# PolySummit/SCORP

Hardware: AMD Instinct MI355X
Metric: fwd+bwd views/sec @1M Gaussians 1600x1200 SH3 (higher is better)
Workload: dtype f32; 1 GPU; S3: 1000000 Gaussians, 1600x1200, SH degree 3, ring cameras (SURVEY 8d); views_per_rank=116, distinct_cameras_per_rank=280, views_in_flight=1, pairs_per_view_D=2428534, visible=966997, parallelism=view-sharded replicas x1

## Files before the change

### scorp_amd/csrc/loss.hip

```cpp
#include "common.hpp"

namespace scorp {
namespace {

constexpr int kLT = 32;
constexpr int kLH = 5;
constexpr int kLP = kLT + 2 * kLH;
constexpr int kLPS = kLP + 3;
constexpr int kLHS = kLT + 1;
constexpr int kHO = 6;
constexpr int kHG = (kLT + kHO - 1) / kHO;
constexpr float kC1 = 0.01f * 0.01f, kC2 = 0.03f * 0.03f;

struct Window { float w[11]; };

Window make_window() {
  Window win;
  float s = 0.0f;
  for (int i = 0; i < 11; i++) { win.w[i] = (float)exp(-(double)((i - 5) * (i - 5)) / (2.0 * 1.5 * 1.5)); s += win.w[i]; }
  for (int i = 0; i < 11; i++) win.w[i] /= s;
  return win;
}

__device__ __forceinline__ float block_sum_256(float v, float *s_red) {
#pragma unroll
  for (int off = 32; off >= 1; off >>= 1) v += __shfl_xor(v, off, 64);
  const int wave = threadIdx.x >> 6;
  __syncthreads();
  if ((threadIdx.x & 63) == 0) s_red[wave] = v;
  __syncthreads();
  return s_red[0] + s_red[1] + s_red[2] + s_red[3];
}

struct LossTile { int ch, x0, y0, logical; bool valid; };
__device__ __forceinline__ LossTile loss_tile(int gx, int gy, int C) {
  const int total = gx * gy * C, per = (total + 7) / 8;
  const int b = blockIdx.x, logical = (b & 7) * per + (b >> 3);
  LossTile t;
  t.valid = (b >> 3) < per && logical < total;
  t.logical = logical;
  t.ch = logical / (gx * gy);
  const int rem = logical - t.ch * gx * gy;
  t.y0 = (rem / gx) * kLT; t.x0 = (rem % gx) * kLT;
  return t;
}

#ifndef SCORP_LOSS_STRIP_ITERS
#define SCORP_LOSS_STRIP_ITERS 3
#endif
constexpr int kStripIters = SCORP_LOSS_STRIP_ITERS;
constexpr int kStripRows = 11 * kStripIters - 10;
constexpr int kRowBuf = 80;

struct StripJob { int ch, cx0, ry0; bool valid; };
__device__ __forceinline__ StripJob strip_job(int C, int H, int W) {
  const int sx = (W + 63) / 64, sy = (H + kStripRows - 1) / kStripRows;
  const int wave = blockIdx.x * 4 + __builtin_amdgcn_readfirstlane((int)(threadIdx.x >> 6));
  StripJob j;
  j.valid = wave < C * sx * sy;
  j.ch = wave / (sx * sy);
  const int rem = wave - j.ch * sx * sy;
  j.ry0 = (rem / sx) * kStripRows; j.cx0 = (rem % sx) * 64;
  return j;
}
static inline int strip_waves(int C, int H, int W) { return C * ((W + 63) / 64) * ((H + kStripRows - 1) / kStripRows); }

__global__ void __launch_bounds__(256)
ssim_l1_forward_strip_kernel(const float *__restrict__ img, const float *__restrict__ gt, const float *__restrict__ mask,
                             int C, int H, int W, Window win, float *__restrict__ dmaps, float *__restrict__ partials) {
  __shared__ __attribute__((aligned(16))) float4 s_row4[4][kRowBuf];
  const StripJob job = strip_job(C, H, W);
  if (!job.valid) return;
  const int lane = threadIdx.x & 63, wv = __builtin_amdgcn_readfirstlane((int)(threadIdx.x >> 6));
  float4 *buf4 = s_row4[wv];
  const int ch = job.ch, cx0 = job.cx0, ry0 = job.ry0;
  const size_t HW = (size_t)H * W, CHW = (size_t)C * HW;
  const float *xp = img + ch * HW, *yp = gt + ch * HW;
  const int gx = cx0 + lane;
  const int ca = cx0 - kLH + lane, cb = cx0 + 64 - kLH + lane;
  const bool cin_a = ca >= 0 && ca < W, cin_b = lane < 2 * kLH && cb < W;
  const int ca_c = min(max(ca, 0), W - 1), cb_c = min(cb, W - 1);
  struct RowRegs { float xa, ya, ma, xb, yb, mb; };
  const uint32_t oa = (uint32_t)ca_c, ob = (uint32_t)cb_c;
  auto fetch = [&](int r) {
    RowRegs v;
    const size_t ro = (size_t)min(max(r, 0), H - 1) * W;
    const float *xr = xp + ro, *yr = yp + ro;
    v.xa = xr[oa]; v.ya = yr[oa]; v.xb = xr[ob]; v.yb = yr[ob];
    v.ma = v.mb = 1.0f;
    if (mask) { const float *mr = mask + ro; v.ma = mr[oa]; v.mb = mr[ob]; }
    return v;
  };
  const int rbeg = ry0 - kLH;
  if (mask) {
    bool any = false;
    {
      constexpr int kSupport = kStripRows + 2 * kLH;
      float ma[kSupport], mb[kSupport];
#pragma unroll
      for (int u = 0; u < kSupport; u++) {
        const float *mr = mask + (size_t)min(max(rbeg + u, 0), H - 1) * W;
        ma[u] = mr[oa]; mb[u] = mr[ob];
      }
#pragma unroll
      for (int u = 0; u < kSupport; u++) any |= (cin_a & (ma[u] != 0.0f)) | (cin_b & (mb[u] != 0.0f));
    }
    if (__ballot(any) == 0) {
      float c1 = kC1, c2 = kC2, zero = 0.0f;
      asm volatile("" : "+v"(c1), "+v"(c2), "+v"(zero));
      const float m1 = zero, m2 = zero, ess = zero, e12 = zero;
      const float m1s = m1 * m1, m2s = m2 * m2, m12 = m1 * m2;
      const float s12 = e12 - m12;
      const float A1 = 2 * m12 + c1, A2 = 2 * s12 + c2, B1 = m1s + m2s + c1, B2 = (ess - m1s - m2s) + c2;
      const float rB2 = __builtin_amdgcn_rcpf(B2);
      const float inv = __builtin_amdgcn_rcpf(B1) * rB2;
      const float ssim = A1 * A2 * inv;
      float ssim_sum = 0.0f;
      for (int ro = ry0; ro < min(ry0 + kStripRows, H); ro++) {
        if (gx < W) {
          ssim_sum += ssim;
          if (dmaps) {
            float *d0 = dmaps + ch * HW + (size_t)ro * W;
            d0[(uint32_t)gx] = (2 * m2 * (A2 - A1) - 2 * m1 * ssim * (B2 - B1)) * inv;
            (d0 + CHW)[(uint32_t)gx] = -ssim * rB2;
            (d0 + 2 * CHW)[(uint32_t)gx] = 2 * A1 * inv;
          }
        }
      }
#pragma unroll
      for (int off = 32; off >= 1; off >>= 1) ssim_sum += __shfl_xor(ssim_sum, off, 64);
      if (lane == 0) {
        const int wave = blockIdx.x * 4 + wv;
        partials[2 * wave] = 0.0f;
        partials[2 * wave + 1] = ssim_sum;
      }
      return;
    }
  }
  float hist[4][11], cx[11], cy[11];
#pragma unroll
  for (int k = 0; k < 11; k++) { hist[0][k] = hist[1][k] = hist[2][k] = hist[3][k] = 0.0f; cx[k] = cy[k] = 0.0f; }
  float l1_sum = 0.0f, ssim_sum = 0.0f;
  RowRegs n0 = fetch(rbeg), n1 = fetch(rbeg + 1);
#pragma unroll 1
  for (int it = 0; it < kStripIters; it++) {
#pragma unroll
    for (int u = 0; u < 11; u++) {
      const int r = rbeg + it * 11 + u;
      const RowRegs cur = n0;
      n0 = n1;
      n1 = fetch(r + 2);
      const bool rin = r >= 0 && r < H;
      {
        const float m = (rin && cin_a) ? cur.ma : 0.0f;
        const float xv = cur.xa * m, yv = cur.ya * m;
        buf4[lane] = make_float4(xv, yv, xv * xv + yv * yv, xv * yv);
        if (lane < 2 * kLH) {
          const float m2 = (rin && cin_b) ? cur.mb : 0.0f;
          const float x2 = cur.xb * m2, y2 = cur.yb * m2;
          buf4[64 + lane] = make_float4(x2, y2, x2 * x2 + y2 * y2, x2 * y2);
        }
      }
      __builtin_amdgcn_fence(__ATOMIC_ACQ_REL, "wavefront");
      __builtin_amdgcn_wave_barrier();
      float h0 = 0, h1 = 0, h2 = 0, h3 = 0;
#pragma unroll
      for (int k = 0; k < 11; k++) {
        const float w = win.w[k];
        const float4 b = buf4[lane + k];
        h0 += w * b.x; h1 += w * b.y; h2 += w * b.z; h3 += w * b.w;
        if (k == kLH) { cx[u] = b.x; cy[u] = b.y; }
      }
      __builtin_amdgcn_fence(__ATOMIC_ACQ_REL, "wavefront");
      __builtin_amdgcn_wave_barrier();
      hist[0][u] = h0; hist[1][u] = h1; hist[2][u] = h2; hist[3][u] = h3;
      const int ro = r - kLH;
      if (ro >= ry0 && ro < H && ro < ry0 + kStripRows) {
        float m1 = 0, m2 = 0, ess = 0, e12 = 0;
#pragma unroll
        for (int k = 0; k < 11; k++) {
          const float w = win.w[k];
          const int sl = (u + 1 + k) % 11;
          m1 += w * hist[0][sl]; m2 += w * hist[1][sl]; ess += w * hist[2][sl]; e12 += w * hist[3][sl];
        }
        if (gx < W) {
          const float m1s = m1 * m1, m2s = m2 * m2, m12 = m1 * m2;
          const float s12 = e12 - m12;
          const float A1 = 2 * m12 + kC1, A2 = 2 * s12 + kC2, B1 = m1s + m2s + kC1, B2 = (ess - m1s - m2s) + kC2;
          const float rB2 = __builtin_amdgcn_rcpf(B2);
          const float inv = __builtin_amdgcn_rcpf(B1) * rB2;
          const float ssim = A1 * A2 * inv;
          ssim_sum += ssim;
          const int sc = (u + 11 - kLH) % 11;
          l1_sum += fabsf(cx[sc] - cy[sc]);
          if (dmaps) {
            float *d0 = dmaps + ch * HW + (size_t)ro * W;
            d0[(uint32_t)gx] = (2 * m2 * (A2 - A1) - 2 * m1 * ssim * (B2 - B1)) * inv;
            (d0 + CHW)[(uint32_t)gx] = -ssim * rB2;
            (d0 + 2 * CHW)[(uint32_t)gx] = 2 * A1 * inv;
          }
        }
      }
    }
  }
#pragma unroll
  for (int off = 32; off >= 1; off >>= 1) { l1_sum += __shfl_xor(l1_sum, off, 64); ssim_sum += __shfl_xor(ssim_sum, off, 64); }
  if (lane == 0) {
    const int wave = blockIdx.x * 4 + wv;
    partials[2 * wave] = l1_sum;
    partials[2 * wave + 1] = ssim_sum;
  }
}

template <int kThreads>
__device__ __forceinline__ void finalize_sums(const float *__restrict__ partials, int nblocks, double n_elems, float lambda,
                                              float *__restrict__ out, double *s_a, double *s_b) {
  const float2 *p2 = reinterpret_cast<const float2 *>(partials);
  double a = 0, b = 0;
  for (int i0 = threadIdx.x; i0 < nblocks; i0 += 4 * kThreads) {
    float2 v[4];
#pragma unroll
    for (int j = 0; j < 4; j++) { const int i = i0 + kThreads * j; v[j] = i < nblocks ? p2[i] : make_float2(0.0f, 0.0f); }
#pragma unroll
    for (int j = 0; j < 4; j++) { a += v[j].x; b += v[j].y; }
  }
  s_a[threadIdx.x] = a; s_b[threadIdx.x] = b;
  __syncthreads();
  for (int off = kThreads / 2; off >= 1; off >>= 1) {
    if ((int)threadIdx.x < off) { s_a[threadIdx.x] += s_a[threadIdx.x + off]; s_b[threadIdx.x] += s_b[threadIdx.x + off]; }
    __syncthreads();
  }
  if (threadIdx.x == 0) {
    const double l1 = s_a[0] / n_elems, ss = s_b[0] / n_elems;
    out[0] = (float)((1.0 - lambda) * l1 + lambda * (1.0 - ss));
    out[1] = (float)l1;
    out[2] = (float)ss;
  }
}

__global__ void __launch_bounds__(1024)
loss_finalize_kernel(const float *__restrict__ partials, int nblocks, double n_elems, float lambda, float *__restrict__ out) {
  __shared__ double s_a[1024], s_b[1024];
  finalize_sums<1024>(partials, nblocks, n_elems, lambda, out, s_a, s_b);
}

struct LossFinalize { const float *partials; int nparts; double n_elems; float *out; };

template <bool kMasked>
__global__ void __launch_bounds__(256)
ssim_l1_backward_kernel(const float *__restrict__ img, const float *__restrict__ gt, const float *__restrict__ mask,
                        const float *__restrict__ dmaps, int C, int H, int W, Window win, float lambda, float inv_n,
                        const float *__restrict__ grad_out, float *__restrict__ grad_img, LossFinalize fin) {
  __shared__ __attribute__((aligned(16))) float s_m[kLP][kLPS];
  __shared__ __attribute__((aligned(16))) float s_h[kLP][kLHS];
  if (fin.out && blockIdx.x == gridDim.x - 1) {
    static_assert(sizeof(s_m) >= 256 * sizeof(double) && sizeof(s_h) >= 256 * sizeof(double), "the tree's scratch fits the tile buffers");
    finalize_sums<256>(fin.partials, fin.nparts, fin.n_elems, lambda, fin.out, reinterpret_cast<double *>(&s_m[0][0]),
                       reinterpret_cast<double *>(&s_h[0][0]));
    return;
  }
  const LossTile lt = loss_tile((W + kLT - 1) / kLT, (H + kLT - 1) / kLT, C);
  if (!lt.valid) return;
  const int ch = lt.ch, x0 = lt.x0, y0 = lt.y0;
  const size_t HW = (size_t)H * W, CHW = (size_t)C * HW;
  const int c = threadIdx.x % kLT, r0 = (threadIdx.x / kLT) * 4;
  const float go = grad_out ? grad_out[0] : 1.0f;
  float xv[4], yv[4], mk[4], acc[4];
  if constexpr (kMasked) {
#pragma unroll
    for (int o = 0; o < 4; o++) {
      const int gy = y0 + r0 + o, gx = x0 + c;
      const float m = mask[(size_t)min(gy, H - 1) * W + min(gx, W - 1)];
      mk[o] = (gy < H && gx < W) ? m : 0.0f;
    }
    const bool any = (mk[0] != 0.0f) | (mk[1] != 0.0f) | (mk[2] != 0.0f) | (mk[3] != 0.0f);
    int *s_any = reinterpret_cast<int *>(&s_h[0][0]);
    if (threadIdx.x == 0) *s_any = 0;
    __syncthreads();
    if (any) *s_any = 1;
    __syncthreads();
    const bool some = *s_any != 0;
    __syncthreads();
    if (!some) {
#pragma unroll
      for (int o = 0; o < 4; o++) {
        const int gy = y0 + r0 + o, gx = x0 + c;
        if (gy < H && gx < W) grad_img[ch * HW + (size_t)gy * W + gx] = 0.0f;
      }
      return;
    }
  } else {
#pragma unroll
    for (int o = 0; o < 4; o++) mk[o] = (y0 + r0 + o < H && x0 + c < W) ? 1.0f : 0.0f;
  }
#pragma unroll
  for (int o = 0; o < 4; o++) {
    const int gy = y0 + r0 + o, gx = x0 + c;
    const size_t p = (size_t)min(gy, H - 1) * W + min(gx, W - 1);
    xv[o] = img[ch * HW + p]; yv[o] = gt[ch * HW + p];
  }
#pragma unroll
  for (int o = 0; o < 4; o++) {
    xv[o] *= mk[o]; yv[o] *= mk[o];
    acc[o] = 0.0f;
  }
  constexpr int kPerThread = (kLP * kLP + 255) / 256;
  float pre[kPerThread];
  auto fetch = [&](int q) {
    const float *map = dmaps + q * CHW + ch * HW;
#pragma unroll
    for (int j = 0; j < kPerThread; j++) {
      const int i = min(threadIdx.x + 256 * j, kLP * kLP - 1);
      const int r = i / kLP, cc = i - r * kLP;
      const int gy = y0 + r - kLH, gx = x0 + cc - kLH;
      pre[j] = map[(size_t)min(max(gy, 0), H - 1) * W + min(max(gx, 0), W - 1)];
    }
  };
  bool pre_in[kPerThread];
#pragma unroll
  for (int j = 0; j < kPerThread; j++) {
    const int i = min(threadIdx.x + 256 * j, kLP * kLP - 1);
    const int r = i / kLP, cc = i - r * kLP;
    const int gy = y0 + r - kLH, gx = x0 + cc - kLH;
    pre_in[j] = gy >= 0 && gy < H && gx >= 0 && gx < W;
  }
  fetch(0);
#pragma unroll 1
  for (int q = 0; q < 3; q++) {
#pragma unroll
    for (int j = 0; j < kPerThread; j++) {
      const int i = threadIdx.x + 256 * j;
      if (i < kLP * kLP) s_m[i / kLP][i % kLP] = pre_in[j] ? pre[j] : 0.0f;
    }
    if (q < 2) fetch(q + 1);
    __syncthreads();
    {
      const int it = threadIdx.x;
      const int r = it / kHG, c0 = (it % kHG) * kHO;
      if (it < kLP * kHG) {
        float v[kHO + 10];
#pragma unroll
        for (int k = 0; k < kHO + 10; k++) v[k] = c0 + k < kLP ? s_m[r][c0 + k] : 0.0f;
#pragma unroll
        for (int o = 0; o < kHO; o++) {
          float sacc = 0;
#pragma unroll
          for (int k = 0; k < 11; k++) sacc += win.w[k] * v[o + k];
          if (c0 + o < kLT) s_h[r][c0 + o] = sacc;
        }
      }
    }
    __syncthreads();
    float col[14];
#pragma unroll
    for (int k = 0; k < 14; k++) col[k] = s_h[r0 + k][c];
#pragma unroll
    for (int o = 0; o < 4; o++) {
      float cv = 0;
#pragma unroll
      for (int k = 0; k < 11; k++) cv += win.w[k] * col[o + k];
      acc[o] += q == 0 ? cv : (q == 1 ? 2.0f * xv[o] * cv : yv[o] * cv);
    }
  }
#pragma unroll
  for (int o = 0; o < 4; o++) {
    const int gy = y0 + r0 + o, gx = x0 + c;
    if (gy < H && gx < W) {
      const float diff = xv[o] - yv[o];
      const float sgn = diff > 0.0f ? 1.0f : (diff < 0.0f ? -1.0f : 0.0f);
      const float g = (1.0f - lambda) * sgn - lambda * acc[o];
      grad_img[ch * HW + (size_t)gy * W + gx] = go * inv_n * mk[o] * g;
    }
  }
}

}
}

using namespace scorp;

static inline int loss_blocks(int C, int H, int W) { return ((W + kLT - 1) / kLT) * ((H + kLT - 1) / kLT) * C; }

extern "C" size_t scorp_loss_workspace_bytes(int32_t C, int32_t H, int32_t W) {
  return align_up((size_t)3 * C * H * W * 4, 256) + align_up((size_t)strip_waves(C, H, W) * 8, 256);
}

namespace scorp {
int loss_forward_impl(const float *img, const float *gt, const float *mask, int32_t C, int32_t H, int32_t W, float lambda_dssim,
                      float *out_loss3, void *workspace, size_t workspace_bytes, int32_t need_backward, bool finalize,
                      hipStream_t stream) {
  if (!img || !gt || !out_loss3 || !workspace) { set_error("NULL argument to scorp_loss_l1_ssim_forward"); return SCORP_ERR_INVALID; }
  if (C <= 0 || H <= 0 || W <= 0) { set_error("bad image shape"); return SCORP_ERR_INVALID; }
  if (workspace_bytes < scorp_loss_workspace_bytes(C, H, W) || ((uintptr_t)workspace & 15)) {
    set_error("loss workspace too small or misaligned"); return SCORP_ERR_INVALID;
  }
  float *dmaps = (float *)workspace;
  float *partials = (float *)((char *)workspace + align_up((size_t)3 * C * H * W * 4, 256));
  const Window win = make_window();
  const int nparts = strip_waves(C, H, W);
  {
    ProfScope prof(kKLossForward, stream);
    ssim_l1_forward_strip_kernel<<<(nparts + 3) / 4, 256, 0, stream>>>(img, gt, mask, C, H, W, win, need_backward ? dmaps : nullptr, partials);
  }
  SCORP_KERNEL_CHECK("ssim_l1_forward", 0, stream);
  if (finalize) {
    loss_finalize_kernel<<<1, 1024, 0, stream>>>(partials, nparts, (double)C * H * W, lambda_dssim, out_loss3);
    SCORP_KERNEL_CHECK("loss_finalize", 0, stream);
  }
  return SCORP_OK;
}

int loss_backward_impl(const float *img, const float *gt, const float *mask, int32_t C, int32_t H, int32_t W, float lambda_dssim,
                       const void *workspace, const float *grad_out, float *grad_img, float *out_loss3, hipStream_t stream) {
  if (!img || !gt || !workspace || !grad_img) { set_error("NULL argument to scorp_loss_l1_ssim_backward"); return SCORP_ERR_INVALID; }
  const int grid = (loss_blocks(C, H, W) + 7) / 8 * 8;
  const Window win = make_window();
  LossFinalize fin;
  fin.partials = (const float *)((const char *)workspace + align_up((size_t)3 * C * H * W * 4, 256));
  fin.nparts = strip_waves(C, H, W);
  fin.n_elems = (double)C * H * W;
  fin.out = out_loss3;
  {
    ProfScope prof(kKLossBackward, stream);
    if (mask)
      ssim_l1_backward_kernel<true><<<grid + (out_loss3 ? 1 : 0), 256, 0, stream>>>(img, gt, mask, (const float *)workspace, C, H, W, win,
                                                                           lambda_dssim, (float)(1.0 / ((double)C * H * W)), grad_out,
                                                                           grad_img, fin);
    else
      ssim_l1_backward_kernel<false><<<grid + (out_loss3 ? 1 : 0), 256, 0, stream>>>(img, gt, mask, (const float *)workspace, C, H, W, win,
                                                                           lambda_dssim, (float)(1.0 / ((double)C * H * W)), grad_out,
                                                                           grad_img, fin);
  }
  SCORP_KERNEL_CHECK("ssim_l1_backward", 0, stream);
  return SCORP_OK;
}
}

extern "C" int scorp_loss_l1_ssim_forward(const float *img, const float *gt, const float *mask, int32_t C, int32_t H,
                                          int32_t W, float lambda_dssim, float *out_loss3, void *workspace,
                                          size_t workspace_bytes, int32_t need_backward, scorp_stream_t stream_) {
  return loss_forward_impl(img, gt, mask, C, H, W, lambda_dssim, out_loss3, workspace, workspace_bytes, need_backward, true,
                           (hipStream_t)stream_);
}

extern "C" int scorp_loss_l1_ssim_backward(const float *img, const float *gt, const float *mask, int32_t C, int32_t H,
                                           int32_t W, float lambda_dssim, const void *workspace, const float *grad_out,
                                           float *grad_img, scorp_stream_t stream_) {
  return loss_backward_impl(img, gt, mask, C, H, W, lambda_dssim, workspace, grad_out, grad_img, nullptr, (hipStream_t)stream_);
}
```

Baseline: 1386 views/s.

## Rewrite SSIM backward as per-wave row-streaming strip kernel with rolling history

```diff
diff --git a/scorp_amd/csrc/loss.hip b/scorp_amd/csrc/loss.hip
--- a/scorp_amd/csrc/loss.hip
+++ b/scorp_amd/csrc/loss.hip
@@ -3,13 +3,7 @@
 namespace scorp {
 namespace {
 
-constexpr int kLT = 32;
 constexpr int kLH = 5;
-constexpr int kLP = kLT + 2 * kLH;
-constexpr int kLPS = kLP + 3;
-constexpr int kLHS = kLT + 1;
-constexpr int kHO = 6;
-constexpr int kHG = (kLT + kHO - 1) / kHO;
 constexpr float kC1 = 0.01f * 0.01f, kC2 = 0.03f * 0.03f;
 
 struct Window { float w[11]; };
@@ -32,19 +26,6 @@
   return s_red[0] + s_red[1] + s_red[2] + s_red[3];
 }
 
-struct LossTile { int ch, x0, y0, logical; bool valid; };
-__device__ __forceinline__ LossTile loss_tile(int gx, int gy, int C) {
-  const int total = gx * gy * C, per = (total + 7) / 8;
-  const int b = blockIdx.x, logical = (b & 7) * per + (b >> 3);
-  LossTile t;
-  t.valid = (b >> 3) < per && logical < total;
-  t.logical = logical;
-  t.ch = logical / (gx * gy);
-  const int rem = logical - t.ch * gx * gy;
-  t.y0 = (rem / gx) * kLT; t.x0 = (rem % gx) * kLT;
-  return t;
-}
-
 #ifndef SCORP_LOSS_STRIP_ITERS
 #define SCORP_LOSS_STRIP_ITERS 3
 #endif
@@ -53,9 +34,9 @@
 constexpr int kRowBuf = 80;
 
 struct StripJob { int ch, cx0, ry0; bool valid; };
-__device__ __forceinline__ StripJob strip_job(int C, int H, int W) {
+__device__ __forceinline__ StripJob strip_job(int wg, int C, int H, int W) {
   const int sx = (W + 63) / 64, sy = (H + kStripRows - 1) / kStripRows;
-  const int wave = blockIdx.x * 4 + __builtin_amdgcn_readfirstlane((int)(threadIdx.x >> 6));
+  const int wave = wg * 4 + __builtin_amdgcn_readfirstlane((int)(threadIdx.x >> 6));
   StripJob j;
   j.valid = wave < C * sx * sy;
   j.ch = wave / (sx * sy);
@@ -69,7 +50,7 @@
 ssim_l1_forward_strip_kernel(const float *__restrict__ img, const float *__restrict__ gt, const float *__restrict__ mask,
                              int C, int H, int W, Window win, float *__restrict__ dmaps, float *__restrict__ partials) {
   __shared__ __attribute__((aligned(16))) float4 s_row4[4][kRowBuf];
-  const StripJob job = strip_job(C, H, W);
+  const StripJob job = strip_job(blockIdx.x, C, H, W);
   if (!job.valid) return;
   const int lane = threadIdx.x & 63, wv = __builtin_amdgcn_readfirstlane((int)(threadIdx.x >> 6));
   float4 *buf4 = s_row4[wv];
@@ -247,130 +228,133 @@
 struct LossFinalize { const float *partials; int nparts; double n_elems; float *out; };
 
 template <bool kMasked>
-__global__ void __launch_bounds__(256)
+__global__ void __launch_bounds__(256, kMasked ? 5 : 6)
 ssim_l1_backward_kernel(const float *__restrict__ img, const float *__restrict__ gt, const float *__restrict__ mask,
                         const float *__restrict__ dmaps, int C, int H, int W, Window win, float lambda, float inv_n,
                         const float *__restrict__ grad_out, float *__restrict__ grad_img, LossFinalize fin) {
-  __shared__ __attribute__((aligned(16))) float s_m[kLP][kLPS];
-  __shared__ __attribute__((aligned(16))) float s_h[kLP][kLHS];
+  __shared__ __attribute__((aligned(16))) float4 s_row4[4][kRowBuf];
   if (fin.out && blockIdx.x == gridDim.x - 1) {
-    static_assert(sizeof(s_m) >= 256 * sizeof(double) && sizeof(s_h) >= 256 * sizeof(double), "the tree's scratch fits the tile buffers");
-    finalize_sums<256>(fin.partials, fin.nparts, fin.n_elems, lambda, fin.out, reinterpret_cast<double *>(&s_m[0][0]),
-                       reinterpret_cast<double *>(&s_h[0][0]));
+    static_assert(sizeof(s_row4) >= 2 * 256 * sizeof(double), "the tree's scratch fits the row buffers");
+    double *s_tree = reinterpret_cast<double *>(&s_row4[0][0]);
+    finalize_sums<256>(fin.partials, fin.nparts, fin.n_elems, lambda, fin.out, s_tree, s_tree + 256);
     return;
   }
-  const LossTile lt = loss_tile((W + kLT - 1) / kLT, (H + kLT - 1) / kLT, C);
-  if (!lt.valid) return;
-  const int ch = lt.ch, x0 = lt.x0, y0 = lt.y0;
+  const int nwg = (C * ((W + 63) / 64) * ((H + kStripRows - 1) / kStripRows) + 3) / 4, per = (nwg + 7) / 8;
+  const int logical = ((int)blockIdx.x & 7) * per + ((int)blockIdx.x >> 3);
+  if (((int)blockIdx.x >> 3) >= per || logical >= nwg) return;
+  const StripJob job = strip_job(logical, C, H, W);
+  if (!job.valid) return;
+  const int lane = threadIdx.x & 63, wv = __builtin_amdgcn_readfirstlane((int)(threadIdx.x >> 6));
+  float4 *buf4 = s_row4[wv];
+  const int ch = job.ch, cx0 = job.cx0, ry0 = job.ry0;
   const size_t HW = (size_t)H * W, CHW = (size_t)C * HW;
-  const int c = threadIdx.x % kLT, r0 = (threadIdx.x / kLT) * 4;
+  const float *xp = img + ch * HW, *yp = gt + ch * HW, *dp = dmaps + ch * HW;
+  float *gp = grad_img + ch * HW;
+  const int gx = cx0 + lane;
+  const int ca = cx0 - kLH + lane, bq = min(lane / (2 * kLH), 2), bc = min(lane - bq * (2 * kLH), 2 * kLH - 1), cb = cx0 + 64 - kLH + bc;
+  const bool cin_a = ca >= 0 && ca < W, cin_b = lane < 6 * kLH && cb < W;
+  const uint32_t oa = 4u * (uint32_t)min(max(ca, 0), W - 1), og = 4u * (uint32_t)min(gx, W - 1);
+  auto at = [](const float *row, uint32_t byte_off) -> const float & {
+    asm("" : "+s"(row));
+    typedef const __attribute__((address_space(1))) char *GlobalBytes;
+    return *(const float *)((GlobalBytes)row + byte_off);
+  };
+  const size_t ob = (size_t)bq * CHW + (size_t)min(cb, W - 1);
+  float *bufb = reinterpret_cast<float *>(buf4 + 64 + bc) + bq;
+  const int rows = min(kStripRows, H - ry0);
+  uint32_t live = (2u << ((rows + 9) / 11)) - 1u;
+  if constexpr (kMasked) {
+    float mv[kStripRows];
+#pragma unroll
+    for (int j = 0; j < kStripRows; j++) mv[j] = at(mask + (size_t)min(ry0 + j, H - 1) * W, og);
+    bool nz[kStripIters];
+#pragma unroll
+    for (int i = 0; i < kStripIters; i++) nz[i] = false;
+#pragma unroll
+    for (int j = 0; j < kStripRows; j++) nz[(j + 10) / 11] |= (j < rows) & (gx < W) & (mv[j] != 0.0f);
+    live = 0;
+#pragma unroll
+    for (int i = 0; i < kStripIters; i++) live |= __ballot(nz[i]) != 0 ? 1u << i : 0u;
+#pragma unroll
+    for (int j = 0; j < kStripRows; j++)
+      if (!((live >> ((j + 10) / 11)) & 1u) && j < rows && gx < W) const_cast<float &>(at(gp + (size_t)(ry0 + j) * W, og)) = 0.0f;
+    if (live == 0) return;
+  }
+  const uint32_t feeds = live | (live >> 1);
+  const int it_lo = kMasked ? __builtin_ctz(feeds) : 0, it_hi = 31 - __builtin_clz(live);
+  struct RowRegs { float a0, a1, a2, b, x, y, m; };
+  auto fetch = [&](int r) {
+    RowRegs v;
+    const float *mr = dp + (size_t)min(max(r, 0), H - 1) * W;
+    v.a0 = at(mr, oa); v.a1 = at(mr + CHW, oa); v.a2 = at(mr + 2 * CHW, oa);
+    v.b = mr[ob];
+    const size_t po = (size_t)min(max(r - kLH, 0), H - 1) * W;
+    v.x = at(xp + po, og); v.y = at(yp + po, og);
+    v.m = 1.0f;
+    if constexpr (kMasked) v.m = at(mask + po, og);
+    return v;
+  };
+  auto uniform = [](float v) {
+    asm("" : "+v"(v));
+    return __builtin_bit_cast(float, __builtin_amdgcn_readfirstlane(__builtin_bit_cast(int, v)));
+  };
   const float go = grad_out ? grad_out[0] : 1.0f;
-  float xv[4], yv[4], mk[4], acc[4];
-  if constexpr (kMasked) {
-#pragma unroll
-    for (int o = 0; o < 4; o++) {
-      const int gy = y0 + r0 + o, gx = x0 + c;
-      const float m = mask[(size_t)min(gy, H - 1) * W + min(gx, W - 1)];
-      mk[o] = (gy < H && gx < W) ? m : 0.0f;
+  const float gscale = uniform(go * inv_n), one_m_lambda = uniform(1.0f - lambda);
+  float hist[3][11];
+#pragma unroll
+  for (int k = 0; k < 11; k++) hist[0][k] = hist[1][k] = hist[2][k] = 0.0f;
+  const int rbeg = ry0 - kLH;
+  RowRegs n0 = fetch(rbeg + 11 * it_lo), n1 = fetch(rbeg + 11 * it_lo + 1);
+#pragma unroll 1
+  for (int it = it_lo; it <= it_hi; it++) {
+    const bool out_it = !kMasked || ((live >> it) & 1u);
+#pragma unroll
+    for (int u = 0; u < 11; u++) {
+      const int r = rbeg + it * 11 + u;
+      const RowRegs cur = n0;
+      n0 = n1;
+      n1 = fetch(r + 2);
+      const bool rin = r >= 0 && r < H;
+      {
+        const bool in_a = rin && cin_a;
+        buf4[lane] = make_float4(in_a ? cur.a0 : 0.0f, in_a ? cur.a1 : 0.0f, in_a ? cur.a2 : 0.0f, 0.0f);
+        if (lane < 6 * kLH) *bufb = (rin && cin_b) ? cur.b : 0.0f;
+      }
+      __builtin_amdgcn_fence(__ATOMIC_ACQ_REL, "wavefront");
+      __builtin_amdgcn_wave_barrier();
+      float h0 = 0.0f, h1 = 0.0f, h2 = 0.0f;
+#pragma unroll
+      for (int k = 0; k < 11; k++) {
+        const float w = win.w[k];
+        const float4 b = buf4[lane + k];
+        h0 = __builtin_fmaf(w, b.x, h0); h1 = __builtin_fmaf(w, b.y, h1); h2 = __builtin_fmaf(w, b.z, h2);
+      }
+      __builtin_amdgcn_fence(__ATOMIC_ACQ_REL, "wavefront");
+      __builtin_amdgcn_wave_barrier();
+      hist[0][u] = h0; hist[1][u] = h1; hist[2][u] = h2;
+      const int ro = r - kLH;
+      if (out_it && ro >= ry0 && ro < ry0 + rows) {
+        float va = 0.0f, vb = 0.0f, vd = 0.0f;
+#pragma unroll
+        for (int k = 0; k < 11; k++) {
+          const float w = win.w[k];
+          const int sl = (u + 1 + k) % 11;
+          va = __builtin_fmaf(w, hist[0][sl], va); vb = __builtin_fmaf(w, hist[1][sl], vb); vd = __builtin_fmaf(w, hist[2][sl], vd);
+        }
+        if (gx < W) {
+#pragma clang fp contract(off)
+          const float xv = cur.x * cur.m, yv = cur.y * cur.m;
+          float acc = 0.0f;
+          acc += va;
+          acc += 2.0f * xv * vb;
+          acc += yv * vd;
+          const float diff = xv - yv;
+          const float sgn = diff > 0.0f ? 1.0f : (diff < 0.0f ? -1.0f : 0.0f);
+          const float g = __builtin_fmaf(one_m_lambda, sgn, -(lambda * acc));
+          const_cast<float &>(at(gp + (size_t)ro * W, og)) = gscale * cur.m * g;
+        }
+      }
     }
-    const bool any = (mk[0] != 0.0f) | (mk[1] != 0.0f) | (mk[2] != 0.0f) | (mk[3] != 0.0f);
-    int *s_any = reinterpret_cast<int *>(&s_h[0][0]);
-    if (threadIdx.x == 0) *s_any = 0;
-    __syncthreads();
-    if (any) *s_any = 1;
-    __syncthreads();
-    const bool some = *s_any != 0;
-    __syncthreads();
-    if (!some) {
-#pragma unroll
-      for (int o = 0; o < 4; o++) {
-        const int gy = y0 + r0 + o, gx = x0 + c;
-        if (gy < H && gx < W) grad_img[ch * HW + (size_t)gy * W + gx] = 0.0f;
-      }
-      return;
-    }
-  } else {
-#pragma unroll
-    for (int o = 0; o < 4; o++) mk[o] = (y0 + r0 + o < H && x0 + c < W) ? 1.0f : 0.0f;
-  }
-#pragma unroll
-  for (int o = 0; o < 4; o++) {
-    const int gy = y0 + r0 + o, gx = x0 + c;
-    const size_t p = (size_t)min(gy, H - 1) * W + min(gx, W - 1);
-    xv[o] = img[ch * HW + p]; yv[o] = gt[ch * HW + p];
-  }
-#pragma unroll
-  for (int o = 0; o < 4; o++) {
-    xv[o] *= mk[o]; yv[o] *= mk[o];
-    acc[o] = 0.0f;
-  }
-  constexpr int kPerThread = (kLP * kLP + 255) / 256;
-  float pre[kPerThread];
-  auto fetch = [&](int q) {
-    const float *map = dmaps + q * CHW + ch * HW;
-#pragma unroll
-    for (int j = 0; j < kPerThread; j++) {
-      const int i = min(threadIdx.x + 256 * j, kLP * kLP - 1);
-      const int r = i / kLP, cc = i - r * kLP;
-      const int gy = y0 + r - kLH, gx = x0 + cc - kLH;
-      pre[j] = map[(size_t)min(max(gy, 0), H - 1) * W + min(max(gx, 0), W - 1)];
-    }
-  };
-  bool pre_in[kPerThread];
-#pragma unroll
-  for (int j = 0; j < kPerThread; j++) {
-    const int i = min(threadIdx.x + 256 * j, kLP * kLP - 1);
-    const int r = i / kLP, cc = i - r * kLP;
-    const int gy = y0 + r - kLH, gx = x0 + cc - kLH;
-    pre_in[j] = gy >= 0 && gy < H && gx >= 0 && gx < W;
-  }
-  fetch(0);
-#pragma unroll 1
-  for (int q = 0; q < 3; q++) {
-#pragma unroll
-    for (int j = 0; j < kPerThread; j++) {
-      const int i = threadIdx.x + 256 * j;
-      if (i < kLP * kLP) s_m[i / kLP][i % kLP] = pre_in[j] ? pre[j] : 0.0f;
-    }
-    if (q < 2) fetch(q + 1);
-    __syncthreads();
-    {
-      const int it = threadIdx.x;
-      const int r = it / kHG, c0 = (it % kHG) * kHO;
-      if (it < kLP * kHG) {
-        float v[kHO + 10];
-#pragma unroll
-        for (int k = 0; k < kHO + 10; k++) v[k] = c0 + k < kLP ? s_m[r][c0 + k] : 0.0f;
-#pragma unroll
-        for (int o = 0; o < kHO; o++) {
-          float sacc = 0;
-#pragma unroll
-          for (int k = 0; k < 11; k++) sacc += win.w[k] * v[o + k];
-          if (c0 + o < kLT) s_h[r][c0 + o] = sacc;
-        }
-      }
-    }
-    __syncthreads();
-    float col[14];
-#pragma unroll
-    for (int k = 0; k < 14; k++) col[k] = s_h[r0 + k][c];
-#pragma unroll
-    for (int o = 0; o < 4; o++) {
-      float cv = 0;
-#pragma unroll
-      for (int k = 0; k < 11; k++) cv += win.w[k] * col[o + k];
-      acc[o] += q == 0 ? cv : (q == 1 ? 2.0f * xv[o] * cv : yv[o] * cv);
-    }
-  }
-#pragma unroll
-  for (int o = 0; o < 4; o++) {
-    const int gy = y0 + r0 + o, gx = x0 + c;
-    if (gy < H && gx < W) {
-      const float diff = xv[o] - yv[o];
-      const float sgn = diff > 0.0f ? 1.0f : (diff < 0.0f ? -1.0f : 0.0f);
-      const float g = (1.0f - lambda) * sgn - lambda * acc[o];
-      grad_img[ch * HW + (size_t)gy * W + gx] = go * inv_n * mk[o] * g;
-    }
   }
 }
 
@@ -378,8 +362,6 @@
 }
 
 using namespace scorp;
-
-static inline int loss_blocks(int C, int H, int W) { return ((W + kLT - 1) / kLT) * ((H + kLT - 1) / kLT) * C; }
 
 extern "C" size_t scorp_loss_workspace_bytes(int32_t C, int32_t H, int32_t W) {
   return align_up((size_t)3 * C * H * W * 4, 256) + align_up((size_t)strip_waves(C, H, W) * 8, 256);
@@ -413,7 +395,7 @@
 int loss_backward_impl(const float *img, const float *gt, const float *mask, int32_t C, int32_t H, int32_t W, float lambda_dssim,
                        const void *workspace, const float *grad_out, float *grad_img, float *out_loss3, hipStream_t stream) {
   if (!img || !gt || !workspace || !grad_img) { set_error("NULL argument to scorp_loss_l1_ssim_backward"); return SCORP_ERR_INVALID; }
-  const int grid = (loss_blocks(C, H, W) + 7) / 8 * 8;
+  const int grid = ((strip_waves(C, H, W) + 3) / 4 + 7) / 8 * 8;
   const Window win = make_window();
   LossFinalize fin;
   fin.partials = (const float *)((const char *)workspace + align_up((size_t)3 * C * H * W * 4, 256));
```

After: 1388 views/s, median of 4. No clear change (+0.1%).
